# qq456cvb/CPPF

Measured on AMD Instinct MI355X. Metric: point-pairs/sec (PPF+MLP+vote+argmax), N=4096 K=128; 1/2/4/8 GPU, higher is better.
Workload: dtype f32; 1 GPU; c2: single object N=4096 K=128 (P=524288 pairs), bottle config, res 0.004, grid 26x76x26, num_rots 72 adaptive, fused PPF+MLP(MFMA f32)+decode of the  ... (full text: bench_full.json); parallelism=objects x1

## Files before the change

### cppf_amd/csrc/vote.hip

```cpp
#include "vote_common.h"

#define VOTE_MAX_TILES 64
#define VOTE_WIN 72

__host__ __device__ inline int vote_fixed_bits_of(int64_t chunk_pairs, int n_rots)
{
    const double cap = 2048.0 * 4294967296.0 / ((double)(chunk_pairs > 0 ? chunk_pairs : 1) * n_rots) - 4.0;
    int kk = 24;
    while (kk > 8 && (double)(1u << kk) > cap) --kk;
    return kk;
}


static int v3_fixed_bits_bound(int64_t n_ppfs, int n_rots, int gx, int gy, int gz);
static bool v3_eligible(int64_t n_ppfs, int n_rots, int gx, int gy, int gz);
static size_t v3_workspace_bytes(int64_t n_ppfs, int gx, int gy, int gz);
static size_t v3_workspace_bytes_dyn(int many_tiles, int64_t n_ppfs);
static int v3_fused_tiles();
extern "C" int cppf_vote_fixed_point_bits(int64_t n_ppfs, int n_rots, int gx, int gy, int gz)
{
    if (n_rots < 1 || n_rots > CPPF_MAX_ROTS || gx < 1 || gy < 1 || gz < 1 || n_ppfs < 0) return -1;
    return v3_eligible(n_ppfs, n_rots, gx, gy, gz) ? v3_fixed_bits_bound(n_ppfs, n_rots, gx, gy, gz) : 0;
}

extern "C" size_t cppf_vote_workspace_bytes(int64_t n_ppfs, int n_rots, int gx, int gy, int gz)
{
    if (n_rots < 1 || n_rots > CPPF_MAX_ROTS || gx < 1 || gy < 1 || gz < 1 || n_ppfs < 0) return 0;
    if (!v3_eligible(n_ppfs, n_rots, gx, gy, gz)) return cppf_vote_workspace_init_bytes();
    return v3_workspace_bytes(n_ppfs, gx, gy, gz);
}
extern "C" size_t cppf_vote_workspace_bytes_dyn_pairs(int many_tiles, int64_t n_ppfs)
{
    if (n_ppfs < 0) return 0;
    return v3_workspace_bytes_dyn(many_tiles, n_ppfs);
}
#define VOTE_PAIRQ 128
#define VOTE_CARRY_CAP 2048
__device__ __forceinline__ uint32_t rpi_u32(float x)
{
    int r;
    asm("v_cvt_rpi_i32_f32 %0, %1" : "=v"(r) : "v"(x));
    return (uint32_t)r;
}

__device__ __forceinline__ float ceil_to_float(double d)
{
    float f = (float)d;
    if ((double)f < d) f = __uint_as_float(__float_as_uint(f) + (f > 0.f ? 1u : -1u));
    return f;
}

#define VOTE_BELOW_N 97

struct Mask96 { uint32_t a, b, c; };

template <bool WIDE = false>
__device__ __forceinline__ Mask96 arc_run(const uint4* __restrict__ below, int ia, int ib, int n, int L = 0)
{
    int len = ib - ia + 1;
    len = len < 0 ? 0 : len;
    const bool full = len >= n;
    int s0 = ia < 0 ? ia + n : ia;
    s0 = s0 >= n ? s0 - n : s0;
    s0 = full ? 0 : (s0 < 0 ? 0 : s0);
    const int e = full ? n : s0 + len;
    if (WIDE) {
        const uint4 B1 = below[min(e, L)], B0 = below[min(s0, L)], B2 = below[min(max(e - n, 0), L)];
        return {(B1.x & ~B0.x) | B2.x, (B1.y & ~B0.y) | B2.y, (B1.z & ~B0.z) | B2.z};
    }
    const uint4 B1 = below[e < n ? e : n], B0 = below[s0], B2 = below[e > n ? e - n : 0];
    return {(B1.x & ~B0.x) | B2.x, (B1.y & ~B0.y) | B2.y, (B1.z & ~B0.z) | B2.z};
}
__device__ __forceinline__ float arc_shift(float f, int n, int win_base)
{
    const float g = f - (float)win_base;
    return g <= -0.5f * (float)n ? g + (float)n : g;
}

template <bool WIDE = false>
__device__ __forceinline__ Mask96 axis_arc_mask(const uint4* __restrict__ below, float c, float x, float y, float lo, float hi,
                                                float nf, int n, int win_base = 0, int L = 0)
{
    const float A = __builtin_amdgcn_sqrtf(fmaf(x, x, y * y));
    const float rA = __builtin_amdgcn_rcpf(fmaxf(A, 1e-20f));
    const float u1 = fmaf(lo - c, rA, -1e-4f);
    const float u2 = fmaf(hi - c, rA, 1e-4f);
    const bool none = !(u1 <= 1.f) || !(u2 >= -1.f);
    const float a1 = u1 <= -1.f ? 3.14159265f : acos_approx(fminf(u1, 1.f));
    const float a2 = u2 >= 1.f ? 0.f : acos_approx(fmaxf(u2, -1.f));
    float f = atan2_approx(y, x) * nf;
    if (WIDE) f = arc_shift(f, n, win_base);
    const float W1 = (a1 + 2e-3f) * nf, W2 = (a2 - 2e-3f) * nf;
    const Mask96 O = arc_run<WIDE>(below, (int)ceilf(f - W1), (int)floorf(f + W1), n, L);
    const Mask96 I = arc_run<WIDE>(below, (int)floorf(f - W2) + 1, W2 > 0.f ? (int)ceilf(f + W2) - 1 : -(1 << 20), n, L);
    const uint32_t keep = none ? 0u : 0xffffffffu;
    return {O.a & ~I.a & keep, O.b & ~I.b & keep, O.c & ~I.c & keep};
}

__device__ __forceinline__ int ctz96(uint32_t a, uint32_t b, uint32_t c)
{
    const uint32_t f0 = (uint32_t)(__ffs((int)a) - 1), f1 = (uint32_t)(__ffs((int)b) - 1) | 32u, f2 = (uint32_t)(__ffs((int)c) - 1) | 64u;
    return (int)min(min(f0, f1), min(f2, 96u));
}
__device__ __forceinline__ int top96(uint32_t a, uint32_t b, uint32_t c)
{
    const int ea = 32 - __clz((int)a), tb = 32 - __clz((int)b), tc = 32 - __clz((int)c);
    return max(ea, max(tb ? tb + 32 : 0, tc ? tc + 64 : 0));
}
__device__ __forceinline__ void mask_runs(const uint4* __restrict__ below, uint32_t m0, uint32_t m1, uint32_t m2, int& s0, int& e0,
                                          int& s1, int& e1, int& s2, int& e2)
{
    s0 = ctz96(m0, m1, m2);
    uint4 B = below[s0];
    e0 = ctz96(~(m0 | B.x), ~(m1 | B.y), ~(m2 | B.z));
    B = below[e0];
    s1 = ctz96(m0 & ~B.x, m1 & ~B.y, m2 & ~B.z);
    B = below[s1];
    e1 = ctz96(~(m0 | B.x), ~(m1 | B.y), ~(m2 | B.z));
    B = below[e1];
    const uint32_t r0 = m0 & ~B.x, r1 = m1 & ~B.y, r2 = m2 & ~B.z;
    s2 = ctz96(r0, r1, r2);
    e2 = top96(r0, r1, r2);
}
#define RED_GROUPS 16
#define RED_MAX_BLOCKS 256
__global__ __launch_bounds__(64 * RED_GROUPS) void reduce_argmax_kernel(float* __restrict__ grid,
                                                                        const float* __restrict__ partials, int chunks,
                                                                        int64_t G, unsigned long long* packed,
                                                                        int accumulate, int write_back,
                                                                        long long* out_idx, float* out_val)
{
    __shared__ float part[RED_GROUPS][64];
    const int lane = threadIdx.x & 63, cg = threadIdx.x >> 6;
    const int64_t ngroups = (G + 63) / 64;
    unsigned long long key = 0ull;
    for (int64_t grp = blockIdx.x; grp < ngroups; grp += gridDim.x) {
        const int64_t cell = grp * 64 + lane;
        float s = 0.f;
        if (cell < G) {
            int c = cg;
            for (; c + 7 * RED_GROUPS < chunks; c += 8 * RED_GROUPS) {
                float v[8];
#pragma unroll
                for (int k = 0; k < 8; ++k) v[k] = partials[(int64_t)(c + k * RED_GROUPS) * G + cell];
#pragma unroll
                for (int k = 0; k < 8; ++k) s = s + v[k];
            }
            for (; c < chunks; c += RED_GROUPS) s = s + partials[(int64_t)c * G + cell];
        }
        part[cg][lane] = s;
        __syncthreads();
        if (cg == 0 && cell < G) {
            float v = accumulate ? grid[cell] : 0.f;
#pragma unroll
            for (int k = 0; k < RED_GROUPS; ++k) v = v + part[k][lane];
            if (write_back) grid[cell] = v;
            const unsigned long long kk =
                ((unsigned long long)f2ord(v) << 32) | (unsigned long long)(0xffffffffu - (uint32_t)cell);
            key = kk > key ? kk : key;
        }
        __syncthreads();
    }
    if (cg != 0) return;
    key = wave_max_u64(key);
    if (lane == 0) {
        const unsigned long long old = atomicMax(packed, key);
        unsigned d1 = (unsigned)old, d2;
        asm volatile("v_mov_b32 %0, %1" : "=v"(d2) : "v"(d1));
        unsigned* ticket = reinterpret_cast<unsigned*>(packed + 1);
        const unsigned tk = atomicAdd(ticket, 1u + (d1 ^ d2));
        if (tk == gridDim.x - 1) {
            const unsigned long long best = atomicMax(packed, 0ull);
            if (out_idx) *out_idx = (long long)(0xffffffffu - (uint32_t)(best & 0xffffffffull));
            if (out_val) *out_val = ord2f((uint32_t)(best >> 32));
        }
    }
}

#define RED_CELLS 256
#define RED_FANIN 8

#define V3_TILE_FLOATS 30720
#ifndef V3_STAGE
#define V3_STAGE 3072
#endif
#define V3_MAGIC 0x43503356u
#define V3_THREADS 1024
#define V3_BIN_THREADS 512
#define V3_BIN_SR 8
#define V3_IRING 256
#define V3_CNT_STRIDE 32
#define V3_RED_FANIN 16
struct V3Hdr {
    unsigned int tile_count[VOTE_MAX_TILES * V3_CNT_STRIDE];
    unsigned int flags;
    unsigned int any_extra;
    unsigned int magic;
    unsigned int fmt;
    float quantum;
    unsigned int done;
    unsigned int pad[2];
};
#define V3_HDR_BYTES ((sizeof(V3Hdr) + 255) / 256 * 256)
#define V3_PLANE_BYTES ((size_t)VOTE_MAX_TILES * V3_TILE_FLOATS * sizeof(unsigned long long))
static_assert(V3_HDR_BYTES + V3_PLANE_BYTES <= VOTE_WS_V3_STATE, "VOTE_WS_V3_STATE too small");

struct V3Tiling { int tx, ty, ntx, nty, T, hx, hy; };
// ... 919 lines not shown
#ifdef V3_TRACE
    __syncthreads();
    if (tid == 0) trace[3] = wall_clock64();
#endif
}

template <bool FUSED, bool WIDE>
__global__ __launch_bounds__(V3_THREADS) void v3_vote_kernel(V3Args A)
{
    v3_vote_body<FUSED, WIDE>(A, (int)blockIdx.x);
}

#define V3_BATCH_MAX 8
struct V3Batch {
    V3Args item[V3_BATCH_MAX];
    int wg_begin[V3_BATCH_MAX + 1];
    int red_begin[V3_BATCH_MAX + 1];
    int bps[V3_BATCH_MAX];
    int n;
};
static_assert(sizeof(V3Batch) <= 4096, "V3Batch travels by value: kernel arguments are limited to 4 KB");
__global__ __launch_bounds__(V3_THREADS) void v3_vote_batch_kernel(V3Batch B)
{
    int i = 0;
    while (i + 1 < B.n && (int)blockIdx.x >= B.wg_begin[i + 1]) ++i;
    if (B.item[i].fused) v3_vote_body<true, false>(B.item[i], (int)blockIdx.x - B.wg_begin[i]);
    else v3_vote_body<false, false>(B.item[i], (int)blockIdx.x - B.wg_begin[i]);
}

__device__ __forceinline__ void v3_rezero(V3Hdr* h)
{
    for (int k = 0; k < VOTE_MAX_TILES; ++k) h->tile_count[k * V3_CNT_STRIDE] = 0u;
    for (int k = 0; k < V3_RED_FANIN; ++k)
        for (int w = 2; w < 6; ++w) h->tile_count[k * V3_CNT_STRIDE + w] = 0u;
    h->flags = 0u; h->any_extra = 0u; h->done = 0u; h->magic = V3_MAGIC;
    __threadfence();
}
__device__ __forceinline__ void v3_reduce_body(const V3Args& A, const int bps, const int bid, const int nblocks)
{
    __shared__ unsigned long long part[RED_GROUPS][RED_CELLS];
    __shared__ unsigned long long wkey[RED_GROUPS];
    __shared__ int sp[200];
    const int tid = threadIdx.x, lane = tid & 63, cg = tid >> 6;
    if (bid == 0 && tid == 0) {
        const unsigned long long st = A.packed[31];
        if ((st & ~0xfffull) == VOTE_TAB_PENDING) A.packed[31] = st ^ (VOTE_TAB_PENDING ^ VOTE_TAB_STAMP);
    }
    int gx, gy, gz;
    int64_t n_points;
    V3Tiling pt;
    const bool fits = v3_resolve(A, gx, gy, gz, n_points, pt);
    const unsigned hflags = A.hdr->flags, hextra = A.hdr->any_extra, hfmt = A.hdr->fmt, hmagic = A.hdr->magic;
    const float hquantum = A.hdr->quantum;
    if (fits) v3_split(A, pt.T, sp);
    if (!fits || (hflags & 1u)) {
        const bool poisoned = hmagic != 0u && hmagic != V3_MAGIC;
        if (!poisoned) {
            uint4* p4 = reinterpret_cast<uint4*>(A.plane);
            const int64_t n16 = (int64_t)(V3_PLANE_BYTES / 16);
            for (int64_t i = (int64_t)bid * blockDim.x + tid; i < n16; i += (int64_t)nblocks * blockDim.x) p4[i] = make_uint4(0u, 0u, 0u, 0u);
            __threadfence();
            __syncthreads();
        }
        if (tid == 0) {
            const unsigned tk = atomicAdd(reinterpret_cast<unsigned*>(A.packed + 18), 1u);
            if (tk == (unsigned)nblocks - 1u) {
                if (A.out_idx) *A.out_idx = -1;
                if (A.out_val) *A.out_val = __uint_as_float(0x7fc00000u);
                if (A.quantum_out) *A.quantum_out = 0.f;
                A.packed[20] = 1ull;
                if (!poisoned) v3_rezero(A.hdr);
            }
        }
        return;
    }
    const bool earlier_pass_failed = A.win_base > 0 && A.packed[20] != 0ull;
    if (A.quantum_out && bid == 0 && tid == 0) *A.quantum_out = (hfmt == 0u && !earlier_pass_failed) ? hquantum : 0.f;
    const int T = pt.T;
    const int slot = v3_slot_words(pt, gz);
    __syncthreads();
    const bool raw = hfmt == 0u;
    const bool any_extra = hextra != 0u;
    unsigned long long best = 0ull;
    const bool wave_items = !A.fused && A.wgs <= 128;
    if (wave_items) {
        for (int item = bid * RED_GROUPS + cg; item < T * bps; item += nblocks * RED_GROUPS) {
            const int t = item / bps, j = item - t * bps;
            const int tix = t / pt.nty, tiy = t - tix * pt.nty;
            const int x0 = tix * pt.tx, y0 = tiy * pt.ty;
            const int tx = min(pt.tx, gx - x0), ty = min(pt.ty, gy - y0);
            const int tyh = pt.ty + pt.hy, ltyz = tyh * gz;
            const int nwords = (tx + pt.hx) * ltyz;
            const int k0 = j * RED_CELLS + lane * 4;
            if (k0 >= nwords) continue;
            const int C = sp[t], base_b = sp[64 + t];
            const unsigned n_own = (unsigned)sp[128 + t];
            unsigned long long acc[4] = {0ull, 0ull, 0ull, 0ull};
            float facc[4] = {0.f, 0.f, 0.f, 0.f};
            const uint32_t* base = A.partials + (int64_t)base_b * slot + k0;
            auto add = [&](const uint4 v) {
                if (raw) { acc[0] += v.x; acc[1] += v.y; acc[2] += v.z; acc[3] += v.w; }
                else { facc[0] += __uint_as_float(v.x); facc[1] += __uint_as_float(v.y); facc[2] += __uint_as_float(v.z); facc[3] += __uint_as_float(v.w); }
            };
            const bool full = n_own >= 64u * (unsigned)C;
            int c = 0;
            if (full) {
                for (; c + 3 < C; c += 4) {
                    uint4 v[4];
#pragma unroll
                    for (int q = 0; q < 4; ++q) v[q] = *reinterpret_cast<const uint4*>(base + (int64_t)(c + q) * slot);
#pragma unroll
                    for (int q = 0; q < 4; ++q) add(v[q]);
                }
            }
            for (; c < C; ++c)
                if (full || v3_chunk_live(n_own, c, C, base_b + c)) add(*reinterpret_cast<const uint4*>(base + (int64_t)c * slot));
#pragma unroll
            for (int u = 0; u < 4; ++u) {
                const int k = k0 + u;
                if (k >= nwords) continue;
                const int lx = k / ltyz, rem = k - lx * ltyz, ly = rem / gz, z = rem - ly * gz;
                if (!(lx < tx && ly < ty)) continue;
                const int64_t cell = ((int64_t)(x0 + lx) * gy + (y0 + ly)) * gz + z;
                const unsigned long long ext = any_extra ? A.plane[cell] : 0ull;
                if (ext) A.plane[cell] = 0ull;
                float v;
                if (raw) {
                    const unsigned long long s_ = ext + acc[u];
                    if (A.grid_raw) A.grid_raw[cell] = (long long)s_ + (A.accumulate ? A.grid_raw[cell] : 0ll);
                    v = (float)((double)s_ * (double)hquantum);
                } else {
                    v = __uint_as_float((uint32_t)ext) + facc[u];
                }
                if (A.accumulate && A.grid) v = A.grid[cell] + v;
                if (A.grid) A.grid[cell] = v;
                const unsigned long long key = ((unsigned long long)f2ord(v) << 32) | (unsigned long long)(0xffffffffu - (uint32_t)cell);
                best = key > best ? key : best;
            }
        }
    } else
    for (int item = bid; item < T * bps; item += nblocks) {
    const int t = item / bps, j = item - t * bps;
    const int tix = t / pt.nty, tiy = t - tix * pt.nty;
    const int x0 = tix * pt.tx, y0 = tiy * pt.ty;
    const int tx = min(pt.tx, gx - x0), ty = min(pt.ty, gy - y0);
    const int tyh = pt.ty + pt.hy, ltyz = tyh * gz;
    const int nwords = (tx + pt.hx) * ltyz;
    if (j * RED_CELLS >= nwords) continue;
    const int C = sp[t], base_b = sp[64 + t];
    const unsigned n_own = (unsigned)sp[128 + t];

    const int k0 = j * RED_CELLS + lane * 4;
    unsigned long long acc[4] = {0ull, 0ull, 0ull, 0ull};
    float facc[4] = {0.f, 0.f, 0.f, 0.f};
    if (k0 < nwords) {
        const uint32_t* base = A.partials + (int64_t)base_b * slot + k0;
        auto add = [&](const uint4 v) {
            if (raw) { acc[0] += v.x; acc[1] += v.y; acc[2] += v.z; acc[3] += v.w; }
            else { facc[0] += __uint_as_float(v.x); facc[1] += __uint_as_float(v.y); facc[2] += __uint_as_float(v.z); facc[3] += __uint_as_float(v.w); }
        };
        const int64_t cp = 64;
        const bool full = A.fused ? (int64_t)(C - 1) * cp < A.n_ppfs : n_own >= 64u * (unsigned)C;
        int c = cg;
        if (full) {
            for (; c + 7 * RED_GROUPS < C; c += 8 * RED_GROUPS) {
                uint4 v[8];
#pragma unroll
                for (int q = 0; q < 8; ++q) v[q] = *reinterpret_cast<const uint4*>(base + (int64_t)(c + q * RED_GROUPS) * slot);
#pragma unroll
                for (int q = 0; q < 8; ++q) add(v[q]);
            }
        }
        for (; c < C; c += RED_GROUPS)
            if (full || (A.fused ? (base_b + c == 0 || (int64_t)c * cp < A.n_ppfs) : v3_chunk_live(n_own, c, C, base_b + c)))
                add(*reinterpret_cast<const uint4*>(base + (int64_t)c * slot));
    }
#pragma unroll
    for (int u = 0; u < 4; ++u) part[cg][lane * 4 + u] = raw ? acc[u] : (unsigned long long)__float_as_uint(facc[u]);

    const int k = j * RED_CELLS + tid;
    int lx = 0, ly = 0, z = 0;
    bool owned = false;
    if (tid < RED_CELLS && k < nwords) {
        lx = k / ltyz;
        const int rem = k - lx * ltyz;
        ly = rem / gz; z = rem - ly * gz;
        owned = lx < tx && ly < ty;
    }
    const int64_t cell = ((int64_t)(x0 + lx) * gy + (y0 + ly)) * gz + z;
    unsigned long long ext = 0ull;
    float prev = 0.f;
    if (owned && any_extra) ext = A.plane[cell];
    if (owned && A.accumulate && A.grid) prev = A.grid[cell];
    __syncthreads();
    if (owned) {
        float v;
        if (ext) A.plane[cell] = 0ull;
        if (raw) {
            unsigned long long s_ = ext;
#pragma unroll
            for (int g = 0; g < RED_GROUPS; ++g) s_ += part[g][tid];
            if (A.grid_raw) A.grid_raw[cell] = (long long)s_ + (A.accumulate ? A.grid_raw[cell] : 0ll);
            v = (float)((double)s_ * (double)hquantum);
        } else {
            v = __uint_as_float((uint32_t)ext);
#pragma unroll
            for (int g = 0; g < RED_GROUPS; ++g) v = v + __uint_as_float((uint32_t)part[g][tid]);
        }
        if (A.accumulate) v = prev + v;
        if (A.grid) A.grid[cell] = v;
        const unsigned long long key = ((unsigned long long)f2ord(v) << 32) | (unsigned long long)(0xffffffffu - (uint32_t)cell);
        best = key > best ? key : best;
    }
    __syncthreads();
    }
    unsigned long long key = best;
    const int n_wkeys = wave_items ? RED_GROUPS : RED_CELLS / 64;
    if (cg < n_wkeys) {
        key = wave_max_u64(key);
        if (lane == 0) wkey[cg] = key;
    }
    const unsigned gsel = (unsigned)bid & (V3_RED_FANIN - 1);
// ... 19 lines not shown
            }
        }
    }
}

__global__ __launch_bounds__(64 * RED_GROUPS) void v3_reduce_kernel(V3Args A, int bps)
{
    v3_reduce_body(A, bps, (int)blockIdx.x, (int)gridDim.x);
}
__global__ __launch_bounds__(64 * RED_GROUPS) void v3_reduce_batch_kernel(V3Batch B)
{
    int i = 0;
    while (i + 1 < B.n && (int)blockIdx.x >= B.red_begin[i + 1]) ++i;
    v3_reduce_body(B.item[i], B.bps[i], (int)blockIdx.x - B.red_begin[i], B.red_begin[i + 1] - B.red_begin[i]);
}

extern "C" size_t cppf_vote_workspace_init_bytes(void)
{
    return VOTE_WS_PART + V3_HDR_BYTES + V3_PLANE_BYTES;
}

static bool v3_eligible(int64_t n_ppfs, int n_rots, int gx, int gy, int gz)
{
    (void)n_rots;
    if (n_ppfs < 1 || n_ppfs > 0xffffffffll) return false;
    return v3_tiling(gx, gy, gz).T <= VOTE_MAX_TILES;
}
static int v3_fixed_bits_bound(int64_t n_ppfs, int n_rots, int gx, int gy, int gz)
{
    const V3Tiling t = v3_tiling(gx, gy, gz);
    const int wgs = v3_wgs(n_ppfs, t.T);
    if (t.T < v3_fused_tiles()) return v3_bits((unsigned)v3_fused_bits_pairs(n_ppfs, wgs / t.T, t.T), n_rots);
    const int wref = wgs < V3_BITS_WGS ? wgs : V3_BITS_WGS;
    const int64_t E = wref - t.T;
    const int64_t worst = E > 0 ? min(n_ppfs, (n_ppfs * t.T + E - 1) / E + 1) : n_ppfs;
    return v3_bits((unsigned)(worst > 0x7fffffff ? 0x7fffffff : worst), n_rots);
}
static size_t v3_workspace_bytes(int64_t n_ppfs, int gx, int gy, int gz)
{
    const V3Tiling t = v3_tiling(gx, gy, gz);
    return v3_plan(n_ppfs, t, gz, v3_wgs(n_ppfs, t.T), t.T < 4 ? 0 : n_ppfs, (int64_t)gx * gy * gz).total;
}
static inline int v3_dyn_tcap(int many_tiles)
{
    return many_tiles == 0 ? 3 : (many_tiles < 4 || many_tiles > VOTE_MAX_TILES ? VOTE_MAX_TILES : many_tiles);
}
static size_t v3_workspace_bytes_dyn(int many_tiles, int64_t n_ppfs)
{
    const int t_cap = v3_dyn_tcap(many_tiles), wgs = V3_WGS;
    return VOTE_WS_PART + V3_HDR_BYTES + V3_PLANE_BYTES +
           (many_tiles ? align_up((size_t)t_cap * (size_t)n_ppfs * 12, 256) + align_up((size_t)n_ppfs * V3_FRAME_BYTES, 256) : 0) +
           (size_t)wgs * V3_TILE_FLOATS * sizeof(uint32_t);
}
extern "C" int cppf_vote_plan_query(int64_t n_ppfs, int n_rots, int gx, int gy, int gz, int32_t* out)
{
    if (!out || n_rots < 1 || n_rots > CPPF_MAX_ROTS || gx < 1 || gy < 1 || gz < 1 || n_ppfs < 0) return CPPF_EINVAL;
    for (int k = 0; k < 10; ++k) out[k] = 0;
    if (v3_eligible(n_ppfs, n_rots, gx, gy, gz)) {
        const V3Tiling t = v3_tiling(gx, gy, gz);
        int wgs = v3_wgs(n_ppfs, t.T);
        if (t.T < v3_fused_tiles()) wgs = (wgs / t.T) * t.T;
        const int o[10] = {t.T < v3_fused_tiles() ? 2 : 3, t.T, t.tx, t.ty, t.ntx, t.nty, t.hx, t.hy, wgs, v3_fixed_bits_bound(n_ppfs, n_rots, gx, gy, gz)};
        for (int k = 0; k < 10; ++k) out[k] = o[k];
        return 0;
    }
    return 0;
}

struct VoteExtras { long long* grid_raw; float* quantum_out; int fixed_bits; };

#define V3_FUSED_TILES 4
static int v3_fused_tiles()
{
    static int v = 0;
    if (v == 0) {
        const char* e = getenv("CPPF_FUSED_MAX_TILES");
        const int w = e ? atoi(e) : V3_FUSED_TILES;
        v = w < V3_FUSED_TILES ? V3_FUSED_TILES : (w > VOTE_MAX_TILES + 1 ? VOTE_MAX_TILES + 1 : w);
    }
    return v;
}

struct V3Launch { V3Args A; int red_blocks, bps; };

static int v3_prepare(V3Launch& Lc, const float* points, const float* outputs, const float* probs, const void* point_idxs, int idx_is_i64,
                      float* grid_obj, const float* corner, float res, int64_t n_points, int64_t n_ppfs, int n_rots, int gx, int gy,
                      int gz, int adaptive, int accumulate, bool want_argmax, long long* out_idx, float* out_val, void* workspace,
                      const int32_t* shape_dev, int64_t grid_cap, int many_tiles, const VoteExtras* ex, int wg_cap, int wg_floor = V3_BITS_WGS)
{
    const int wgs_max = wg_cap > 0 ? (wg_cap < wg_floor ? wg_floor : (wg_cap > V3_WGS ? V3_WGS : wg_cap)) : V3_WGS;
    char* ws = static_cast<char*>(workspace);
    V3Args& A = Lc.A;
    A = V3Args{};
    if (ex) { A.grid_raw = ex->grid_raw; A.quantum_out = ex->quantum_out; A.kk_force = ex->fixed_bits; }
    A.points = points; A.outputs = outputs; A.probs = probs; A.point_idxs = point_idxs; A.idx64 = idx_is_i64;
    A.corner = corner; A.res = res; A.n_ppfs = n_ppfs; A.n_points = n_points; A.n_rots = n_rots; A.adaptive = adaptive;
    A.gx = gx; A.gy = gy; A.gz = gz; A.shape = shape_dev; A.grid_cap = grid_cap;
    A.hdr = reinterpret_cast<V3Hdr*>(ws + VOTE_WS_PART);
    A.packed = reinterpret_cast<unsigned long long*>(ws);
    A.grid = grid_obj; A.accumulate = accumulate;
    A.out_idx = want_argmax ? out_idx : nullptr; A.out_val = want_argmax ? out_val : nullptr;
    const bool wide = n_rots > VOTE_WIN;
    A.tab_entries = wide ? 0 : tri(n_rots);
    A.pool_cap = n_ppfs;
    A.plane = reinterpret_cast<unsigned long long*>(ws + VOTE_WS_PART + V3_HDR_BYTES);
    if (shape_dev) {
        A.t_cap = v3_dyn_tcap(many_tiles);
        A.wgs = wgs_max;
        A.fused = many_tiles ? 0 : 1;
        if (ex && ex->grid_raw) return CPPF_EINVAL;
        if (grid_cap > (int64_t)A.t_cap * V3_TILE_FLOATS) return CPPF_EINVAL;
        A.pool = reinterpret_cast<uint32_t*>(ws + VOTE_WS_PART + V3_HDR_BYTES + V3_PLANE_BYTES);
        A.frames = reinterpret_cast<float4*>(A.pool + (many_tiles ? align_up((size_t)A.t_cap * (size_t)n_ppfs * 12, 256) / 4 : 0));
        A.partials = reinterpret_cast<uint32_t*>(A.frames) + (many_tiles ? align_up((size_t)n_ppfs * V3_FRAME_BYTES, 256) / 4 : 0);
        const int bps = ((V3_TILE_FLOATS + RED_CELLS - 1) / RED_CELLS + RED_FANIN - 1) / RED_FANIN * RED_FANIN;
        Lc.red_blocks = A.t_cap * bps;
    } else {
        A.t = v3_tiling(gx, gy, gz);
        A.wgs = v3_wgs(n_ppfs, A.t.T);
        if (A.wgs > wgs_max) A.wgs = wgs_max > A.t.T ? wgs_max : A.t.T;
        A.fused = A.t.T < v3_fused_tiles() ? 1 : 0;
        if (A.fused) {
            A.wgs = (A.wgs / A.t.T) * A.t.T;
            A.kk = v3_bits((unsigned)v3_fused_bits_pairs(n_ppfs, A.wgs / A.t.T, A.t.T), n_rots);
        }
        A.t_cap = A.t.T;
        const V3Plan pl = v3_plan(n_ppfs, A.t, gz, v3_wgs(n_ppfs, A.t.T), A.fused ? 0 : n_ppfs, (int64_t)gx * gy * gz);
        A.pool = reinterpret_cast<uint32_t*>(ws + pl.pool_off);
        A.frames = reinterpret_cast<float4*>(ws + pl.frames_off);
        A.partials = reinterpret_cast<uint32_t*>(ws + pl.part_off);
        const int bps = ((pl.slot + RED_CELLS - 1) / RED_CELLS + RED_FANIN - 1) / RED_FANIN * RED_FANIN;
        Lc.red_blocks = A.t.T * bps;
    }
    Lc.bps = Lc.red_blocks / A.t_cap;
    return 0;
}

static size_t v3_vote_lds(const V3Args& A) { return V3_LDS_HEAD + (size_t)(A.tab_entries + 2) * sizeof(float2) + (size_t)V3_TILE_FLOATS * sizeof(float); }
static void v3_set_attrs()
{
    static bool attr_done = false;
    if (!attr_done) {
        const void* ks[] = {reinterpret_cast<const void*>(&v3_bin_kernel<false>), reinterpret_cast<const void*>(&v3_bin_kernel<true>),
                            reinterpret_cast<const void*>(&v3_vote_kernel<false, false>), reinterpret_cast<const void*>(&v3_vote_kernel<true, false>),
                            reinterpret_cast<const void*>(&v3_vote_kernel<false, true>), reinterpret_cast<const void*>(&v3_vote_kernel<true, true>),
                            reinterpret_cast<const void*>(&v3_vote_batch_kernel)};
        for (const void* k : ks) (void)hipFuncSetAttribute(k, hipFuncAttributeMaxDynamicSharedMemorySize, 160 * 1024);
        attr_done = true;
    }
}

static size_t v3_bin_geometry(V3Args& A, dim3& bin_grid)
{
    int64_t srb = A.n_ppfs / ((int64_t)V3_BIN_THREADS * 512);
    srb = srb < 1 ? 1 : (srb > V3_BIN_SR ? V3_BIN_SR : srb);
    A.bin_sr = (int)srb;
    const int64_t rounds = (A.n_ppfs + V3_BIN_THREADS * srb - 1) / (V3_BIN_THREADS * srb);
    bin_grid = dim3((unsigned)(rounds < 512 ? rounds : 512));
    return (size_t)V3_STAGE * 16 + VOTE_BELOW_N * 16 + 2 * VOTE_MAX_TILES * 4 + 64 + (V3_BIN_THREADS / 64) * (V3_IRING * 2 + (64 * V3_BIN_SR + 64) * 4);
}

static int v3_launch(const float* points, const float* outputs, const float* probs, const void* point_idxs, int idx_is_i64,
                     float* grid_obj, const float* corner, float res, int64_t n_points, int64_t n_ppfs, int n_rots, int gx, int gy,
                     int gz, int adaptive, int accumulate, bool want_argmax, long long* out_idx, float* out_val, void* workspace,
                     hipStream_t st, const int32_t* shape_dev, int64_t grid_cap, int many_tiles, const VoteExtras* ex = nullptr,
                     int wg_cap = 0)
{
    V3Launch Lc;
    const int rc = v3_prepare(Lc, points, outputs, probs, point_idxs, idx_is_i64, grid_obj, corner, res, n_points, n_ppfs, n_rots, gx, gy, gz,
                              adaptive, accumulate, want_argmax, out_idx, out_val, workspace, shape_dev, grid_cap, many_tiles, ex, wg_cap);
    if (rc != 0) return rc;
    V3Args& A = Lc.A;
    const int red_blocks = Lc.red_blocks;
    const bool wide = n_rots > VOTE_WIN;
    v3_set_attrs();
    const size_t lds_vote = v3_vote_lds(A);
    dim3 bin_grid;
    const size_t lds_bin = v3_bin_geometry(A, bin_grid);
    const int bps = Lc.bps;
    const dim3 red_grid((unsigned)(red_blocks < 2 * V3_WGS ? red_blocks : 2 * V3_WGS));
    if (wide && A.grid_raw && !A.kk_force) A.kk_force = v3_fixed_bits_bound(n_ppfs, n_rots, gx, gy, gz);
    for (int wb = 0; wb < n_rots; wb += VOTE_WIN) {
        A.win_base = wb;
        if (wb > 0) A.accumulate = 1;
        if (A.fused) {
            if (wide) hipLaunchKernelGGL((v3_vote_kernel<true, true>), dim3((unsigned)A.wgs), dim3(V3_THREADS), lds_vote, st, A);
            else hipLaunchKernelGGL((v3_vote_kernel<true, false>), dim3((unsigned)A.wgs), dim3(V3_THREADS), lds_vote, st, A);
            CPPF_CHECK_LAUNCH();
        } else {
            if (wide) hipLaunchKernelGGL(v3_bin_kernel<true>, bin_grid, dim3(V3_BIN_THREADS), lds_bin, st, A);
            else hipLaunchKernelGGL(v3_bin_kernel<false>, bin_grid, dim3(V3_BIN_THREADS), lds_bin, st, A);
            CPPF_CHECK_LAUNCH();
            if (wide) hipLaunchKernelGGL((v3_vote_kernel<false, true>), dim3((unsigned)A.wgs), dim3(V3_THREADS), lds_vote, st, A);
            else hipLaunchKernelGGL((v3_vote_kernel<false, false>), dim3((unsigned)A.wgs), dim3(V3_THREADS), lds_vote, st, A);
            CPPF_CHECK_LAUNCH();
        }
        hipLaunchKernelGGL(v3_reduce_kernel, red_grid, dim3(64 * RED_GROUPS), 0, st, A, bps);
        CPPF_CHECK_LAUNCH();
    }
    return 0;
}

__global__ void zero_u64x2_kernel(unsigned long long* p) { p[0] = 0ull; p[1] = 0ull; }
__global__ void set_f32_kernel(float* p, float v) { *p = v; }

__global__ __launch_bounds__(256) void vote_global_kernel(const float* __restrict__ points, const float* __restrict__ outputs,
                                                          const float* __restrict__ probs, const void* __restrict__ point_idxs, int idx64,
                                                          float* __restrict__ grid, const float* __restrict__ corner, float res,
                                                          int64_t n_ppfs, int n_rots, int gx, int gy, int gz, int adaptive)
{
    const f3 cr = {corner[0], corner[1], corner[2]};
    const int64_t syz = (int64_t)gy * gz;
    for (int64_t p = (int64_t)blockIdx.x * blockDim.x + threadIdx.x; p < n_ppfs; p += (int64_t)gridDim.x * blockDim.x) {
        const float2 o = reinterpret_cast<const float2*>(outputs)[p];
        int2 ij;
        if (idx64) { const longlong2 v = reinterpret_cast<const longlong2*>(point_idxs)[p]; ij = make_int2((int)v.x, (int)v.y); }
        else ij = reinterpret_cast<const int2*>(point_idxs)[p];
        f3 a, ab, xd;
        if (!pair_frame(points, ij.x, ij.y, a, ab, xd)) continue;
        const f3 cc = sub3(a, scl3(ab, o.x));
        const float prob = probs ? fmaxf(probs[ij.x], probs[ij.y]) : 1.f;
        const f3 x = scl3(xd, o.y), y = cross3(x, ab);
        int n = n_rots;
        if (adaptive) n = min((int)((double)(o.y / res) * (2 * CPPF_PI)), n_rots);
        for (int i = 0; i < n; ++i) {
            const float2 cs = rot_cs(i, n);
            const f3 v = sub3(add3(cc, add3(scl3(x, cs.x), scl3(y, cs.y))), cr);
            const f3 g = {v.x / res, v.y / res, v.z / res};
            if ((double)g.x < 0.01 || (double)g.y < 0.01 || (double)g.z < 0.01 || (double)g.x >= (double)gx - 1.01 ||
                (double)g.y >= (double)gy - 1.01 || (double)g.z >= (double)gz - 1.01) continue;
            const int fx = (int)g.x, fy = (int)g.y, fz = (int)g.z;
            const float rx = g.x - floorf(g.x), ry = g.y - floorf(g.y), rz = g.z - floorf(g.z);
            const float w0x = 1.f - rx, w0y = 1.f - ry, w0z = 1.f - rz;
            float* b = grid + ((int64_t)fx * syz + (int64_t)fy * gz + fz);
            atomicAdd(b, w0x * w0y * w0z * prob);                 atomicAdd(b + 1, w0x * w0y * rz * prob);
            atomicAdd(b + gz, w0x * ry * w0z * prob);             atomicAdd(b + gz + 1, w0x * ry * rz * prob);
            atomicAdd(b + syz, rx * w0y * w0z * prob);            atomicAdd(b + syz + 1, rx * w0y * rz * prob);
            atomicAdd(b + syz + gz, rx * ry * w0z * prob);        atomicAdd(b + syz + gz + 1, rx * ry * rz * prob);
        }
    }
}

static int vote_impl(const float* points, const float* outputs, const float* probs, const void* point_idxs, int idx_is_i64,
                     float* grid_obj, const float* corner, float res, int64_t n_points, int64_t n_ppfs, int n_rots,
                     int gx, int gy, int gz, int adaptive, int accumulate, bool want_argmax, long long* out_idx, float* out_val,
                     void* workspace, size_t workspace_bytes, hipStream_t st, const int32_t* shape_dev = nullptr,
                     int64_t grid_cap = 0, int many_tiles = 0, const VoteExtras* ex = nullptr)
{
    const int wg_cap = (accumulate >> 8) & 0x1ff;
    if ((accumulate & ~(1 | (0x1ff << 8))) != 0) return CPPF_EINVAL;
    accumulate &= 1;
    if (wg_cap != 0 && ex) return CPPF_EINVAL;
    if (!points || (!grid_obj && !(ex && ex->grid_raw)) || !corner) return CPPF_EINVAL;
    if (n_ppfs > 0 && (!outputs || !point_idxs)) return CPPF_EINVAL;
    if (n_rots < 1 || n_rots > CPPF_MAX_ROTS || gx < 1 || gy < 1 || gz < 1 || n_ppfs < 0 || n_points < 1) return CPPF_EINVAL;
    if ((int64_t)gx * gy * gz > 0x7fffffffll) return CPPF_EINVAL;
    if (shape_dev) {
        if (n_ppfs < 1 || n_ppfs > 0xffffffffll || grid_cap < 1 || grid_cap > 0x7fffffffll) return CPPF_EINVAL;
        if (!workspace || workspace_bytes < v3_workspace_bytes_dyn(many_tiles, n_ppfs)) return CPPF_EWORKSPACE;
        return v3_launch(points, outputs, probs, point_idxs, idx_is_i64, grid_obj, corner, res, n_points, n_ppfs, n_rots, gx, gy, gz,
                         adaptive, accumulate, want_argmax, out_idx, out_val, workspace, st, shape_dev, grid_cap, many_tiles, ex, wg_cap);
    }
    if (v3_eligible(n_ppfs, n_rots, gx, gy, gz)) {
// ... 53 lines not shown
{
    return vote_impl(points, outputs, probs, point_idxs, idx_is_i64, grid_obj, corner, res, n_points, n_ppfs, n_rots, gx, gy, gz,
                     adaptive, accumulate, true, out_idx, out_val, workspace, workspace_bytes, (hipStream_t)stream);
}

extern "C" int cppf_vote_argmax_dyn(const float* points, const float* outputs, const float* probs, const void* point_idxs,
                                    int idx_is_i64, float* grid_obj, int64_t grid_capacity, const float* corner, float res,
                                    int64_t n_points_cap, int64_t n_ppfs, int n_rots, const int32_t* shape_dev, int many_tiles,
                                    int adaptive, int accumulate, long long* out_idx, float* out_val, void* workspace,
                                    size_t workspace_bytes, void* stream)
{
    if (!shape_dev) return CPPF_EINVAL;
    return vote_impl(points, outputs, probs, point_idxs, idx_is_i64, grid_obj, corner, res, n_points_cap, n_ppfs, n_rots, 1, 1, 1,
                     adaptive, accumulate, true, out_idx, out_val, workspace, workspace_bytes, (hipStream_t)stream, shape_dev,
                     grid_capacity, many_tiles);
}

extern "C" int cppf_vote_batch_workgroups(int n_items, int flags)
{
    if (n_items < 1 || n_items > V3_BATCH_MAX) return CPPF_EINVAL;
    const int wg_cap = (flags >> 8) & 0x1ff;
    int w = wg_cap > 0 ? wg_cap : V3_WGS / n_items;
    if (w < V3_BITS_WGS) w = V3_BITS_WGS;
    if (w > V3_WGS) w = V3_WGS;
    return w;
}

extern "C" int cppf_vote_argmax_batch(int n_items, const CppfVoteItem* items, int n_rots, int adaptive, int flags, void* stream)
{
    if (n_items < 1 || n_items > V3_BATCH_MAX || !items) return CPPF_EINVAL;
    if ((flags & ~(1 | (0x1ff << 8))) != 0) return CPPF_EINVAL;
    if (n_rots < 1 || n_rots > CPPF_MAX_ROTS) return CPPF_EINVAL;
    hipStream_t st = (hipStream_t)stream;
    const int accumulate = flags & 1;
    auto shares_the_launch = [&](const CppfVoteItem& it) -> bool {
        const bool dyn = it.shape_dev != nullptr;
        bool batched = n_rots <= VOTE_WIN && it.n_ppfs >= 1 && it.points && it.grid && it.corner && it.outputs && it.point_idxs &&
                       it.out_idx && it.out_val && it.workspace && it.n_points >= 1;
        if (batched && dyn) batched = it.n_ppfs <= 0xffffffffll && it.grid_capacity >= 1 &&
                                      it.grid_capacity <= (int64_t)v3_dyn_tcap(it.many_tiles) * V3_TILE_FLOATS &&
                                      it.workspace_bytes >= v3_workspace_bytes_dyn(it.many_tiles, it.n_ppfs);
        if (batched && !dyn) batched = it.gx >= 1 && it.gy >= 1 && it.gz >= 1 && v3_eligible(it.n_ppfs, n_rots, it.gx, it.gy, it.gz) &&
                                       it.workspace_bytes >= v3_workspace_bytes(it.n_ppfs, it.gx, it.gy, it.gz);
        return batched;
    };
    int n_shared = 0;
    for (int i = 0; i < n_items; ++i) n_shared += shares_the_launch(items[i]) ? 1 : 0;
    const int width = cppf_vote_batch_workgroups(n_shared > 0 ? n_shared : n_items, flags);
    V3Batch B = {};
    int vote_wgs = 0, red_blocks = 0;
    size_t lds_vote = 0;
    for (int i = 0; i < n_items; ++i) {
        const CppfVoteItem& it = items[i];
        const bool dyn = it.shape_dev != nullptr;
        const bool batched = shares_the_launch(it);
        if (!batched) {
            const int rc = dyn ? cppf_vote_argmax_dyn(it.points, it.outputs, it.probs, it.point_idxs, it.idx_is_i64, it.grid, it.grid_capacity,
                                                      it.corner, it.res, it.n_points, it.n_ppfs, n_rots, it.shape_dev, it.many_tiles, adaptive,
                                                      flags, it.out_idx, it.out_val, it.workspace, it.workspace_bytes, stream)
                               : cppf_vote_argmax(it.points, it.outputs, it.probs, it.point_idxs, it.idx_is_i64, it.grid, it.corner, it.res,
                                                  it.n_points, it.n_ppfs, n_rots, it.gx, it.gy, it.gz, adaptive, flags, it.out_idx, it.out_val,
                                                  it.workspace, it.workspace_bytes, stream);
            if (rc != 0) return rc;
            continue;
        }
        V3Launch Lc;
        const int rc = v3_prepare(Lc, it.points, it.outputs, it.probs, it.point_idxs, it.idx_is_i64, it.grid, it.corner, it.res, it.n_points,
                                  it.n_ppfs, n_rots, dyn ? 1 : it.gx, dyn ? 1 : it.gy, dyn ? 1 : it.gz, adaptive, accumulate, true, it.out_idx,
                                  it.out_val, it.workspace, it.shape_dev, dyn ? it.grid_capacity : 0, dyn ? it.many_tiles : 0, nullptr, width);
        if (rc != 0) return rc;
        if (!Lc.A.fused) {
            v3_set_attrs();
            dim3 bin_grid;
            const size_t lds_bin = v3_bin_geometry(Lc.A, bin_grid);
            hipLaunchKernelGGL(v3_bin_kernel<false>, bin_grid, dim3(V3_BIN_THREADS), lds_bin, st, Lc.A);
            CPPF_CHECK_LAUNCH();
        }
        const int k = B.n++;
        B.item[k] = Lc.A;
        B.bps[k] = Lc.bps;
        B.wg_begin[k] = vote_wgs;
        B.red_begin[k] = red_blocks;
        vote_wgs += Lc.A.wgs;
        int rb = 2 * V3_WGS / (n_shared > 0 ? n_shared : n_items);
        rb = rb < 64 ? 64 : rb;
        if (!Lc.A.fused && rb < V3_WGS) rb = V3_WGS;
        red_blocks += Lc.red_blocks < rb ? Lc.red_blocks : rb;
        lds_vote = v3_vote_lds(Lc.A);
    }
    if (B.n == 0) return 0;
    B.wg_begin[B.n] = vote_wgs;
    B.red_begin[B.n] = red_blocks;
    v3_set_attrs();
    hipLaunchKernelGGL(v3_vote_batch_kernel, dim3((unsigned)vote_wgs), dim3(V3_THREADS), lds_vote, st, B);
    CPPF_CHECK_LAUNCH();
    hipLaunchKernelGGL(v3_reduce_batch_kernel, dim3((unsigned)red_blocks), dim3(64 * RED_GROUPS), 0, st, B);
    CPPF_CHECK_LAUNCH();
    return 0;
}

extern "C" int cppf_vote_grid_raw(const float* points, const float* outputs, const float* probs, const void* point_idxs,
                                  int idx_is_i64, long long* grid_raw, float* quantum_out, const float* corner, float res,
                                  int64_t n_points, int64_t n_ppfs, int n_rots, int gx, int gy, int gz, int adaptive, int accumulate,
                                  int fixed_bits, void* workspace, size_t workspace_bytes, void* stream)
{
    if (!grid_raw || !quantum_out || fixed_bits < 0 || (fixed_bits != 0 && (fixed_bits < 8 || fixed_bits > 24))) return CPPF_EINVAL;
    const VoteExtras ex = {grid_raw, quantum_out, fixed_bits};
    return vote_impl(points, outputs, probs, point_idxs, idx_is_i64, nullptr, corner, res, n_points, n_ppfs, n_rots, gx, gy, gz,
                     adaptive, accumulate, false, nullptr, nullptr, workspace, workspace_bytes, (hipStream_t)stream, nullptr, 0, 0, &ex);
}

__global__ __launch_bounds__(256) void grid_from_raw_kernel(const long long* __restrict__ raw, int64_t n, const float* __restrict__ quantum,
                                                            float* __restrict__ grid)
{
    const float q = *quantum;
    for (int64_t i = (int64_t)blockIdx.x * blockDim.x + threadIdx.x; i < n; i += (int64_t)gridDim.x * blockDim.x)
        grid[i] = (q > 0.f && q < INFINITY) ? (float)((double)raw[i] * (double)q)
                                            : (q > 0.f && raw[i] == 0ll ? 0.f : __uint_as_float(0x7fc00000u));
}
extern "C" int cppf_grid_from_raw(const long long* grid_raw, int64_t n, const float* quantum, float* grid, long long* out_idx,
                                  float* out_val, void* workspace, size_t workspace_bytes, void* stream)
{
    if (!grid_raw || !quantum || !grid || n < 1 || n > 0x7fffffffll) return CPPF_EINVAL;
    int64_t nb = (n + 255) / 256;
    hipLaunchKernelGGL(grid_from_raw_kernel, dim3((unsigned)(nb > 2048 ? 2048 : nb)), dim3(256), 0, (hipStream_t)stream, grid_raw, n, quantum, grid);
    CPPF_CHECK_LAUNCH();
    return out_idx ? cppf_grid_argmax(grid, n, out_idx, out_val, workspace, workspace_bytes, stream) : 0;
}

extern "C" int cppf_vote_tile_cells(void) { return V3_TILE_FLOATS; }

extern "C" int cppf_vote_tiles(int gx, int gy, int gz)
{
    if (gx < 1 || gy < 1 || gz < 1) return CPPF_EINVAL;
    const int T = v3_tiling(gx, gy, gz).T;
    return T <= VOTE_MAX_TILES ? T : 0;
}

extern "C" int cppf_grid_argmax(const float* grid, int64_t n, long long* out_idx, float* out_val, void* workspace,
                                size_t workspace_bytes, void* stream)
{
    if (!grid || n < 1 || n > 0x7fffffffll || !out_idx) return CPPF_EINVAL;
    if (!workspace || workspace_bytes < 16) return CPPF_EWORKSPACE;
    hipStream_t st = (hipStream_t)stream;
    unsigned long long* packed = static_cast<unsigned long long*>(workspace);
    hipLaunchKernelGGL(zero_u64x2_kernel, dim3(1), dim3(1), 0, st, packed);
    int64_t nb = (n + 63) / 64;
    if (nb > RED_MAX_BLOCKS) nb = RED_MAX_BLOCKS;
    hipLaunchKernelGGL(reduce_argmax_kernel, dim3((unsigned)nb), dim3(64 * RED_GROUPS), 0, st, const_cast<float*>(grid),
                       (const float*)nullptr, 0, n, packed, 1, 0, out_idx, out_val);
    CPPF_CHECK_LAUNCH();
    return 0;
}

extern "C" int cppf_abi_version(void) { return CPPF_ABI_VERSION; }
extern "C" const char* cppf_error_string(int code)
{
    switch (code) {
    case 0: return "success";
    case CPPF_EINVAL: return "cppf: invalid argument";
    case CPPF_EWORKSPACE: return "cppf: workspace missing or too small";
    case CPPF_EUNSUPPORTED: return "cppf: unsupported layer shape";
    case CPPF_ENONFINITE: return "cppf: the cloud holds non-finite coordinates";
    case CPPF_ECAPACITY: return "cppf: a device-side bound (bin list capacity) was exceeded";
    default: return code > 0 ? hipGetErrorString((hipError_t)code) : "cppf: unknown error";
    }
}
```

Measured before the change: 6.441 billion pairs/s.

## Extend wave-per-item reduction to fused raw path with deeper load batching

The per-wave reduction path now also runs when the vote kernel is fused and the format is raw. The raw specialization is a compile-time template that keeps 16 partial-chunk loads in flight per batch, using a liveness mask in place of per-chunk branches. Loop-invariant values are made wave-uniform with readfirstlane, and the plane reads are issued before the chunk loop. The reduce grid is also capped at V3_WGS when this path is taken. This raises memory-level parallelism for the reduction but adds register pressure and may load dead chunks redundantly.

```diff
diff --git a/cppf_amd/csrc/vote.hip b/cppf_amd/csrc/vote.hip
--- a/cppf_amd/csrc/vote.hip
+++ b/cppf_amd/csrc/vote.hip
@@ -1,4 +1,5 @@
 #include "vote_common.h"
+#include <type_traits>
 
 #define VOTE_MAX_TILES 64
 #define VOTE_WIN 72
@@ -123,6 +124,8 @@
     e2 = top96(r0, r1, r2);
 }
 #define RED_GROUPS 16
+#define RED_FLIGHT 16
+#define V3_RED_WAVE_WGS 128
 #define RED_MAX_BLOCKS 256
 __global__ __launch_bounds__(64 * RED_GROUPS) void reduce_argmax_kernel(float* __restrict__ grid,
                                                                         const float* __restrict__ partials, int chunks,
@@ -1208,9 +1211,11 @@
     const bool raw = hfmt == 0u;
     const bool any_extra = hextra != 0u;
     unsigned long long best = 0ull;
-    const bool wave_items = !A.fused && A.wgs <= 128;
-    if (wave_items) {
-        for (int item = bid * RED_GROUPS + cg; item < T * bps; item += nblocks * RED_GROUPS) {
+    const bool wave_items = A.wgs <= V3_RED_WAVE_WGS && (raw || !A.fused);
+    auto wave_form = [&](auto raw_c) {
+        constexpr bool RAW = decltype(raw_c)::value;
+        constexpr int NF = RAW ? RED_FLIGHT : 4;
+        for (int item = bid + nblocks * __builtin_amdgcn_readfirstlane(cg); item < T * bps; item += nblocks * RED_GROUPS) {
             const int t = item / bps, j = item - t * bps;
             const int tix = t / pt.nty, tiy = t - tix * pt.nty;
             const int x0 = tix * pt.tx, y0 = tiy * pt.ty;
@@ -1219,51 +1224,71 @@
             const int nwords = (tx + pt.hx) * ltyz;
             const int k0 = j * RED_CELLS + lane * 4;
             if (k0 >= nwords) continue;
-            const int C = sp[t], base_b = sp[64 + t];
-            const unsigned n_own = (unsigned)sp[128 + t];
-            unsigned long long acc[4] = {0ull, 0ull, 0ull, 0ull};
-            float facc[4] = {0.f, 0.f, 0.f, 0.f};
-            const uint32_t* base = A.partials + (int64_t)base_b * slot + k0;
-            auto add = [&](const uint4 v) {
-                if (raw) { acc[0] += v.x; acc[1] += v.y; acc[2] += v.z; acc[3] += v.w; }
-                else { facc[0] += __uint_as_float(v.x); facc[1] += __uint_as_float(v.y); facc[2] += __uint_as_float(v.z); facc[3] += __uint_as_float(v.w); }
-            };
-            const bool full = n_own >= 64u * (unsigned)C;
-            int c = 0;
-            if (full) {
-                for (; c + 3 < C; c += 4) {
-                    uint4 v[4];
-#pragma unroll
-                    for (int q = 0; q < 4; ++q) v[q] = *reinterpret_cast<const uint4*>(base + (int64_t)(c + q) * slot);
-#pragma unroll
-                    for (int q = 0; q < 4; ++q) add(v[q]);
-                }
-            }
-            for (; c < C; ++c)
-                if (full || v3_chunk_live(n_own, c, C, base_b + c)) add(*reinterpret_cast<const uint4*>(base + (int64_t)c * slot));
+            const int C = __builtin_amdgcn_readfirstlane(sp[t]), base_b = __builtin_amdgcn_readfirstlane(sp[64 + t]);
+            const unsigned n_own = (unsigned)__builtin_amdgcn_readfirstlane(sp[128 + t]);
+            int cell[4];
+            unsigned long long ext[4];
 #pragma unroll
             for (int u = 0; u < 4; ++u) {
                 const int k = k0 + u;
-                if (k >= nwords) continue;
                 const int lx = k / ltyz, rem = k - lx * ltyz, ly = rem / gz, z = rem - ly * gz;
-                if (!(lx < tx && ly < ty)) continue;
-                const int64_t cell = ((int64_t)(x0 + lx) * gy + (y0 + ly)) * gz + z;
-                const unsigned long long ext = any_extra ? A.plane[cell] : 0ull;
-                if (ext) A.plane[cell] = 0ull;
+                cell[u] = (k < nwords && lx < tx && ly < ty) ? ((x0 + lx) * gy + (y0 + ly)) * gz + z : -1;
+                ext[u] = (cell[u] >= 0 && any_extra) ? A.plane[cell[u]] : 0ull;
+            }
+            unsigned long long acc[4] = {0ull, 0ull, 0ull, 0ull};
+            const uint32_t* base = A.partials + (int64_t)base_b * slot + k0;
+            auto add = [&](const uint4 v) {
+                if (RAW) { acc[0] += v.x; acc[1] += v.y; acc[2] += v.z; acc[3] += v.w; }
+                else {
+                    acc[0] = __float_as_uint(__uint_as_float((uint32_t)acc[0]) + __uint_as_float(v.x));
+                    acc[1] = __float_as_uint(__uint_as_float((uint32_t)acc[1]) + __uint_as_float(v.y));
+                    acc[2] = __float_as_uint(__uint_as_float((uint32_t)acc[2]) + __uint_as_float(v.z));
+                    acc[3] = __float_as_uint(__uint_as_float((uint32_t)acc[3]) + __uint_as_float(v.w));
+                }
+            };
+            const bool full = A.fused ? (int64_t)(C - 1) * 64 < A.n_ppfs : n_own >= 64u * (unsigned)C;
+#pragma nounroll
+            for (int c0 = 0; c0 < C; c0 += NF) {
+                unsigned live = C - c0 >= NF ? (1u << NF) - 1u : (1u << (C - c0)) - 1u;
+                if (!full) {
+#pragma nounroll
+                    for (int q = 0; q < NF && c0 + q < C; ++q) {
+                        const int c = c0 + q;
+                        if (!(A.fused ? (base_b + c == 0 || (int64_t)c * 64 < A.n_ppfs) : v3_chunk_live(n_own, c, C, base_b + c))) live &= ~(1u << q);
+                    }
+                }
+                if (live == 0u) continue;
+                const int c_first = c0 + __builtin_ctz(live);
+                uint4 v[NF];
+#pragma unroll
+                for (int q = 0; q < NF; ++q) v[q] = *reinterpret_cast<const uint4*>(base + (int64_t)(((live >> q) & 1u) ? c0 + q : c_first) * slot);
+#pragma unroll
+                for (int q = 0; q < NF; ++q) {
+                    const uint32_t m = 0u - ((live >> q) & 1u);
+                    add(make_uint4(v[q].x & m, v[q].y & m, v[q].z & m, v[q].w & m));
+                }
+            }
+#pragma unroll
+            for (int u = 0; u < 4; ++u) {
+                if (cell[u] < 0) continue;
+                if (ext[u]) A.plane[cell[u]] = 0ull;
                 float v;
-                if (raw) {
-                    const unsigned long long s_ = ext + acc[u];
-                    if (A.grid_raw) A.grid_raw[cell] = (long long)s_ + (A.accumulate ? A.grid_raw[cell] : 0ll);
+                if (RAW) {
+                    const unsigned long long s_ = ext[u] + acc[u];
+                    if (A.grid_raw) A.grid_raw[cell[u]] = (long long)s_ + (A.accumulate ? A.grid_raw[cell[u]] : 0ll);
                     v = (float)((double)s_ * (double)hquantum);
                 } else {
-                    v = __uint_as_float((uint32_t)ext) + facc[u];
+                    v = __uint_as_float((uint32_t)ext[u]) + __uint_as_float((uint32_t)acc[u]);
                 }
-                if (A.accumulate && A.grid) v = A.grid[cell] + v;
-                if (A.grid) A.grid[cell] = v;
-                const unsigned long long key = ((unsigned long long)f2ord(v) << 32) | (unsigned long long)(0xffffffffu - (uint32_t)cell);
+                if (A.accumulate && A.grid) v = A.grid[cell[u]] + v;
+                if (A.grid) A.grid[cell[u]] = v;
+                const unsigned long long key = ((unsigned long long)f2ord(v) << 32) | (unsigned long long)(0xffffffffu - (uint32_t)cell[u]);
                 best = key > best ? key : best;
             }
         }
+    };
+    if (wave_items) {
+        if (raw) wave_form(std::true_type{}); else wave_form(std::false_type{});
     } else
     for (int item = bid; item < T * bps; item += nblocks) {
     const int t = item / bps, j = item - t * bps;
@@ -1449,6 +1474,10 @@
 }
 
 struct V3Launch { V3Args A; int red_blocks, bps; };
+static int v3_red_blocks(int items, int cap)
+{
+    return items < 1 ? 1 : (items > cap ? cap : items);
+}
 
 static int v3_prepare(V3Launch& Lc, const float* points, const float* outputs, const float* probs, const void* point_idxs, int idx_is_i64,
                       float* grid_obj, const float* corner, float res, int64_t n_points, int64_t n_ppfs, int n_rots, int gx, int gy,
@@ -1545,7 +1574,7 @@
     dim3 bin_grid;
     const size_t lds_bin = v3_bin_geometry(A, bin_grid);
     const int bps = Lc.bps;
-    const dim3 red_grid((unsigned)(red_blocks < 2 * V3_WGS ? red_blocks : 2 * V3_WGS));
+    const dim3 red_grid((unsigned)v3_red_blocks(red_blocks, A.wgs <= V3_RED_WAVE_WGS ? V3_WGS : 2 * V3_WGS));
     if (wide && A.grid_raw && !A.kk_force) A.kk_force = v3_fixed_bits_bound(n_ppfs, n_rots, gx, gy, gz);
     for (int wb = 0; wb < n_rots; wb += VOTE_WIN) {
         A.win_base = wb;
@@ -1765,10 +1794,11 @@
         B.wg_begin[k] = vote_wgs;
         B.red_begin[k] = red_blocks;
         vote_wgs += Lc.A.wgs;
-        int rb = 2 * V3_WGS / (n_shared > 0 ? n_shared : n_items);
+        const bool wave_form = Lc.A.wgs <= V3_RED_WAVE_WGS;
+        int rb = (wave_form ? V3_WGS : 2 * V3_WGS) / (n_shared > 0 ? n_shared : n_items);
         rb = rb < 64 ? 64 : rb;
         if (!Lc.A.fused && rb < V3_WGS) rb = V3_WGS;
-        red_blocks += Lc.red_blocks < rb ? Lc.red_blocks : rb;
+        red_blocks += v3_red_blocks(Lc.red_blocks, rb);
         lds_vote = v3_vote_lds(Lc.A);
     }
     if (B.n == 0) return 0;
```

Result: no change. 6.447 billion pairs/s, median of 2 (+0.1%).
